# ArnaudPel/CamKifu

Measured on AMD Instinct MI355X. Metric: frames/sec on 1920x1080 video + 19x19 stone-grid match % vs reference SGF, higher is better.
Workload: dtype u8+f16x2(f32 accumulate); 1 GPU; 1920x1080 synthetic game film, 256-frame batches resident in HBM, K1-K12 per ...; cnn=f16x2, frames_per_gpu=256, height=1080, width=1920, parallelism=frames of one video dealt x1, lanes_per_gpu=2, batches_in_flight=2

## Files before the change

camkifu_amd/csrc/k_contours.hip:

```cpp
#include <math.h>

#include <algorithm>

#include "ck_common.h"

#include "ck_uf.h"

#pragma clang fp contract(off)

namespace {

constexpr int MAXC_LIMIT = 1 << 17;
constexpr int PEAK_CAP = 1 << 14;
constexpr int NUMANGLE = 180;

struct FrameTab {
    int n_edges;
    int n_border;
    int n_roots;
    int n_hough_pts;
    int n_peaks;
    int overflow;
    int runs_overflow;
    int pad1;
// ... 150 lines not shown
    for (int i = bx * 256 + threadIdx.x; i < ne + h; i += LIST_BLOCKS * 256) {
        if (i < ne) {
            const int p = E[i];
            L[p] = uf_find(L, p);
            if (!e[p + 1]) L[p + 1] = uf_find(L, p + 1);
        } else {
            const int q = (i - ne) * w;
            L[q] = uf_find(L, q);
        }
    }
}

__device__ __forceinline__ bool in_s0(const int32_t* L, int q, int root0)
{
    return L[L[q]] == root0;
}

__device__ __forceinline__ void claim_root(int f, size_t off, int p, int32_t* __restrict__ compid, FrameTab* __restrict__ tab, int maxc,
                                           int32_t* __restrict__ roots, int32_t* __restrict__ aabb)
{
    const int slot = atomicAdd(&tab[f].n_roots, 1);
    if (slot >= maxc) { tab[f].overflow = 1; compid[off + p] = -1; return; }
    compid[off + p] = slot;
    int32_t* fr = roots + (size_t)f * maxc;
    fr[slot] = p;
    int32_t* bb = aabb + ((size_t)f * maxc + slot) * 4;
    bb[0] = 0x7fffffff; bb[1] = -1; bb[2] = 0x7fffffff; bb[3] = -1;
}

__global__ __launch_bounds__(256) void roots_list_kernel(int h, int w, const int32_t* __restrict__ labels,
                                                         int32_t* __restrict__ compid, FrameTab* __restrict__ tab, int maxc,
                                                         int32_t* __restrict__ roots, int32_t* __restrict__ aabb,
                                                         const int32_t* __restrict__ elist)
{
    int f, bx;
    list_frame_block(LIST_BLOCKS, f, bx);
    const int ne = tab[f].n_edges;
    const size_t off = (size_t)f * h * w;
    const int32_t* L = labels + off;
    const int32_t* E = elist + off;
    const int root0 = L[0];
    for (int i = bx * 256 + threadIdx.x; i < ne; i += LIST_BLOCKS * 256) {
        const int p = E[i];
        if (L[p] != p) continue;
        if (!in_s0(L, p - 1, root0)) continue;
        claim_root(f, off, p, compid, tab, maxc, roots, aabb);
    }
}

__device__ __forceinline__ void grow_boxes(bool b, int cslot, int p, int w, int f, int maxc, int32_t* __restrict__ aabb)
{
    unsigned long long todo = __builtin_amdgcn_ballot_w64(b);
    const int y = p / w, x = p - y * w;
    const int lane = threadIdx.x & 63;
    while (todo) {
        const int lead = __builtin_ctzll(todo);
        const int s_lead = __builtin_amdgcn_readlane(cslot, lead);
        const bool mine = b && cslot == s_lead;
        todo &= ~__builtin_amdgcn_ballot_w64(mine);
        int mnx = mine ? x : 0x7fffffff, mxx = mine ? x : -1, mny = mine ? y : 0x7fffffff, mxy = mine ? y : -1;
#pragma unroll
        for (int d = 32; d >= 1; d >>= 1) {
            mnx = min(mnx, __shfl_xor(mnx, d)); mxx = max(mxx, __shfl_xor(mxx, d));
            mny = min(mny, __shfl_xor(mny, d)); mxy = max(mxy, __shfl_xor(mxy, d));
        }
        if (lane == lead) {
            int32_t* bb = aabb + ((size_t)f * maxc + s_lead) * 4;
            if (mnx < uf_load(bb, 0)) atomicMin(bb + 0, mnx);
            if (mxx > uf_load(bb, 1)) atomicMax(bb + 1, mxx);
            if (mny < uf_load(bb, 2)) atomicMin(bb + 2, mny);
            if (mxy > uf_load(bb, 3)) atomicMax(bb + 3, mxy);
        }
    }
}

__global__ __launch_bounds__(256) void border_list_kernel(const uint8_t* __restrict__ ez, int h, int w,
                                                          const int32_t* __restrict__ labels, const int32_t* __restrict__ compid,
                                                          int maxc, FrameTab* __restrict__ tab, int32_t* __restrict__ aabb,
                                                          const int32_t* __restrict__ elist, int32_t* __restrict__ blist)
{
    int f, bx;
    list_frame_block(LIST_BLOCKS, f, bx);
    const int ne = tab[f].n_edges;
    const size_t off = (size_t)f * h * w;
    const uint8_t* e = ez + off;
    const int32_t* L = labels + off;
    const int32_t* E = elist + off;
    int32_t* B = blist + off;
    const int root0 = L[0];
    const int trips = (ne + LIST_BLOCKS * 256 - 1) / (LIST_BLOCKS * 256);
    for (int t = 0; t < trips; t++) {
        const int i = t * LIST_BLOCKS * 256 + bx * 256 + threadIdx.x;
        bool b = false;
        int p = 0, cslot = -1;
        if (i < ne) {
            p = E[i];
            const int q[4] = { p - 1, p + 1, p - w, p + w };
            int ev[4], head[4], top[4];
#pragma unroll
            for (int k = 0; k < 4; k++) ev[k] = e[q[k]];
#pragma unroll
            for (int k = 0; k < 4; k++) head[k] = L[ev[k] ? 0 : q[k]];
#pragma unroll
            for (int k = 0; k < 4; k++) top[k] = L[head[k]];
#pragma unroll
            for (int k = 0; k < 4; k++) b |= !ev[k] && top[k] == root0;
            if (b) {
                cslot = compid[off + L[p]];
                if ((unsigned)cslot >= (unsigned)maxc) b = false;
            }
        }
        grow_boxes(b, cslot, p, w, f, maxc, aabb);
        const int slot = wave_append(&tab[f].n_border, b);
        if (b) B[slot] = p;
    }
}

struct RunTab {
    unsigned long long* bits;
    uint16_t* rank;
    int32_t* rowbase;
    int32_t* rp;
    int w64;
    int cap_e;
    size_t rp_stride;
};

__device__ __forceinline__ bool rt_edge(const unsigned long long* __restrict__ bf, int w64, int y, int x)
{
    return (bf[(size_t)y * w64 + (x >> 6)] >> (x & 63)) & 1ull;
}
__device__ __forceinline__ int rt_run(const unsigned long long* __restrict__ bf, const uint16_t* __restrict__ rk,
                                      const int32_t* __restrict__ rb, int h, int w64, int y, int x)
{
    const size_t wi = (size_t)y * w64 + (x >> 6);
    const int r = (int)rk[wi] + __builtin_popcountll(bf[wi] & ((1ull << (x & 63)) - 1ull));
    return r ? h + rb[y] + r - 1 : y;
}

__device__ __forceinline__ unsigned long long row16_or(unsigned long long v)
{
    uint32_t lo = (uint32_t)v, hi = (uint32_t)(v >> 32);
#define CK_DPP_OR(CTRL)                                                                   \
    lo |= (uint32_t)__builtin_amdgcn_update_dpp(0, (int)lo, CTRL, 0xf, 0xf, true);       \
    hi |= (uint32_t)__builtin_amdgcn_update_dpp(0, (int)hi, CTRL, 0xf, 0xf, true);
    CK_DPP_OR(0xB1)
    CK_DPP_OR(0x4E)
    CK_DPP_OR(0x141)
    CK_DPP_OR(0x140)
#undef CK_DPP_OR
    return ((unsigned long long)hi << 32) | lo;
}

template <int NS>
__global__ __launch_bounds__(256) void prep_runs_kernel(const uint8_t* __restrict__ edges, int h, int w, int32_t* __restrict__ L,
                                                        FrameTab* __restrict__ tab, int32_t* __restrict__ elist, RunTab rt,
                                                        const int* __restrict__ canny_border_flag)
{
    const int lane = threadIdx.x & 63, wv = threadIdx.x >> 6;
    const int y = blockIdx.x * 4 + wv;
    const int f = blockIdx.y;
    const bool row_live = y < h;
    __shared__ int wtotal[4], wbase;
    const bool keep_edge_parents = canny_border_flag != nullptr && canny_border_flag[f] == 0;
    const size_t off = ((size_t)f * h + y) * w;
    const bool row_inner = y > 0 && y < h - 1;
    int32_t* E = elist + (size_t)f * h * w;
    int32_t* rp = rt.rp + (size_t)f * rt.rp_stride;
    const unsigned long long lt = (1ull << lane) - 1ull;
    uint32_t v[NS];
#pragma unroll
    for (int s = 0; s < NS; s++) {
        const int x = 256 * s + 4 * lane;
        v[s] = 0;
        if (x < w && row_inner && row_live) v[s] = *reinterpret_cast<const uint32_t*>(edges + off + x);
    }
    int nib[NS], before[NS];
    int total = 0;
#pragma unroll
    for (int s = 0; s < NS; s++) {
        const int x = 256 * s + 4 * lane;
        int nb = ((v[s] & 0xFFu) ? 1 : 0) | ((v[s] & 0xFF00u) ? 2 : 0) | ((v[s] & 0xFF0000u) ? 4 : 0) | ((v[s] & 0xFF000000u) ? 8 : 0);
        if (x == 0) nb &= ~1;
        if (x + 3 == w - 1) nb &= ~8;
        nib[s] = nb;
        before[s] = total;
        if (__builtin_amdgcn_ballot_w64(nb != 0)) {
            const unsigned long long b0 = __builtin_amdgcn_ballot_w64(nb & 1), b1 = __builtin_amdgcn_ballot_w64(nb & 2);
            const unsigned long long b2 = __builtin_amdgcn_ballot_w64(nb & 4), b3 = __builtin_amdgcn_ballot_w64(nb & 8);
            before[s] += __builtin_popcountll(b0 & lt) + __builtin_popcountll(b1 & lt) +
                         __builtin_popcountll(b2 & lt) + __builtin_popcountll(b3 & lt);
            total += __builtin_popcountll(b0) + __builtin_popcountll(b1) + __builtin_popcountll(b2) + __builtin_popcountll(b3);
        }
    }
    if (lane == 0) wtotal[wv] = total;
    __syncthreads();
    if (threadIdx.x == 0) {
        const int all = wtotal[0] + wtotal[1] + wtotal[2] + wtotal[3];
        wbase = all ? atomicAdd(&tab[f].n_edges, all) : 0;
    }
    __syncthreads();
    if (!row_live) return;
    int base = wbase;
    for (int kk = 0; kk < wv; kk++) base += wtotal[kk];
    base = __builtin_amdgcn_readfirstlane(base);
    const bool nodes_fit = base + total <= rt.cap_e;
    if (!nodes_fit && lane == 0) tab[f].runs_overflow = 1;
    if (lane == 0) {
        rt.rowbase[(size_t)f * h + y] = base;
        rp[y] = 0;
    }
    unsigned long long* bw = rt.bits + ((size_t)f * h + y) * rt.w64;
    uint16_t* rw = rt.rank + ((size_t)f * h + y) * rt.w64;
#pragma unroll
    for (int s = 0; s < NS; s++) {
        const int x = 256 * s + 4 * lane;
        const int nb = nib[s];
        const unsigned long long word = row16_or((unsigned long long)nb << (4 * (lane & 15)));
        if (x < w) {
            if ((lane & 15) == 0) {
                bw[4 * s + (lane >> 4)] = word;
                rw[4 * s + (lane >> 4)] = (uint16_t)before[s];
            }
            if (nb) {
                int slot = base + before[s];
#pragma unroll
                for (int k = 0; k < 4; k++)
                    if (nb & (1 << k)) {
                        const int p = y * w + x + k;
                        E[slot] = p;
                        if (nodes_fit) rp[h + slot] = slot == base + total - 1 ? 0 : h + slot;
                        if (!keep_edge_parents) L[(size_t)f * h * w + p] = p;
                        slot++;
                    }
            }
        }
    }
}

__global__ __launch_bounds__(256) void link_runs_kernel(int h, int w, int32_t* __restrict__ labels, const FrameTab* __restrict__ tab,
                                                        const int32_t* __restrict__ elist, RunTab rt,
                                                        const int* __restrict__ canny_border_flag)
{
    int f, bx;
    list_frame_block(LIST_BLOCKS, f, bx);
    if (tab[f].runs_overflow) return;
    const bool edges_linked = canny_border_flag != nullptr && canny_border_flag[f] == 0;
    const int ne = tab[f].n_edges, w64 = rt.w64;
    int32_t* L = labels + (size_t)f * h * w;
    const int32_t* E = elist + (size_t)f * h * w;
    const unsigned long long* bf = rt.bits + (size_t)f * h * w64;
    const uint16_t* rk = rt.rank + (size_t)f * h * w64;
    const int32_t* rb = rt.rowbase + (size_t)f * h;
    int32_t* rp = rt.rp + (size_t)f * rt.rp_stride;
    for (int i = bx * 256 + threadIdx.x; i < ne; i += LIST_BLOCKS * 256) {
        const int p = E[i];
        const int y = p / w, x = p - y * w;
        const bool e_n = rt_edge(bf, w64, y - 1, x), e_ne = rt_edge(bf, w64, y - 1, x + 1);
        const bool e_e = rt_edge(bf, w64, y, x + 1), e_s = rt_edge(bf, w64, y + 1, x), e_se = rt_edge(bf, w64, y + 1, x + 1);
        if (!edges_linked) {
            if (rt_edge(bf, w64, y, x - 1)) uf_union(L, p, p - 1);
            if (e_n) uf_union(L, p, p - w);
            else {
                if (rt_edge(bf, w64, y - 1, x - 1)) uf_union(L, p, p - w - 1);
                if (e_ne) uf_union(L, p, p - w + 1);
            }
        }
        if (!e_e && !e_ne) uf_union(rp, h + i, rt_run(bf, rk, rb, h, w64, y - 1, x + 1));
        if (!e_se && !e_e && !e_s) uf_union(rp, rt_run(bf, rk, rb, h, w64, y + 1, x + 1), h + i);
    }
}

__global__ __launch_bounds__(256) void flatten_runs_kernel(int h, int w, int32_t* __restrict__ labels, const FrameTab* __restrict__ tab,
                                                           const int32_t* __restrict__ elist, RunTab rt,
                                                           const int* __restrict__ canny_border_flag)
{
    int f, bx;
    list_frame_block(LIST_BLOCKS, f, bx);
    if (tab[f].runs_overflow) return;
    const bool edges_flat = canny_border_flag != nullptr && canny_border_flag[f] == 0;
    const int ne = tab[f].n_edges;
    int32_t* L = labels + (size_t)f * h * w;
    const int32_t* E = elist + (size_t)f * h * w;
    int32_t* rp = rt.rp + (size_t)f * rt.rp_stride;
    for (int i = bx * 256 + threadIdx.x; i < ne + h; i += LIST_BLOCKS * 256) {
        rp[i] = uf_find(rp, i);
        if (!edges_flat && i < ne) { const int p = E[i]; L[p] = uf_find(L, p); }
    }
}

__global__ __launch_bounds__(256) void roots_runs_kernel(int h, int w, const int32_t* __restrict__ labels,
                                                         int32_t* __restrict__ compid, FrameTab* __restrict__ tab, int maxc,
                                                         int32_t* __restrict__ roots, int32_t* __restrict__ aabb,
                                                         const int32_t* __restrict__ elist, RunTab rt)
{
    int f, bx;
    list_frame_block(LIST_BLOCKS, f, bx);
    if (tab[f].runs_overflow) return;
    const int ne = tab[f].n_edges;
    const size_t off = (size_t)f * h * w;
    const int32_t* L = labels + off;
    const int32_t* E = elist + off;
    const int32_t* rb = rt.rowbase + (size_t)f * h;
    const int32_t* rp = rt.rp + (size_t)f * rt.rp_stride;
    const int root0 = rp[0];
    for (int i = bx * 256 + threadIdx.x; i < ne; i += LIST_BLOCKS * 256) {
        const int p = E[i];
        if (L[p] != p) continue;
        const int y = p / w;
        const int west = (i == rb[y]) ? y : h + i - 1;
        if (rp[west] != root0) continue;
        claim_root(f, off, p, compid, tab, maxc, roots, aabb);
    }
}

__global__ __launch_bounds__(256) void border_runs_kernel(int h, int w, const int32_t* __restrict__ labels,
                                                          const int32_t* __restrict__ compid, int maxc, FrameTab* __restrict__ tab,
                                                          int32_t* __restrict__ aabb, const int32_t* __restrict__ elist,
                                                          int32_t* __restrict__ blist, RunTab rt)
{
    int f, bx;
    list_frame_block(LIST_BLOCKS, f, bx);
    if (tab[f].runs_overflow) return;
    const int ne = tab[f].n_edges, w64 = rt.w64;
    const size_t off = (size_t)f * h * w;
    const int32_t* L = labels + off;
    const int32_t* E = elist + off;
    int32_t* B = blist + off;
    const unsigned long long* bf = rt.bits + (size_t)f * h * w64;
    const uint16_t* rk = rt.rank + (size_t)f * h * w64;
    const int32_t* rb = rt.rowbase + (size_t)f * h;
    const int32_t* rp = rt.rp + (size_t)f * rt.rp_stride;
    const int root0 = rp[0];
    const int trips = (ne + LIST_BLOCKS * 256 - 1) / (LIST_BLOCKS * 256);
    for (int t = 0; t < trips; t++) {
        const int i = t * LIST_BLOCKS * 256 + bx * 256 + threadIdx.x;
        bool b = false;
        int p = 0, cslot = -1;
        if (i < ne) {
            p = E[i];
            const int y = p / w, x = p - y * w;
            const size_t wi = (size_t)y * w64 + (x >> 6);
            const unsigned long long here = bf[wi];
            const bool e_w = (x & 63) ? (here >> ((x & 63) - 1)) & 1ull : rt_edge(bf, w64, y, x - 1);
            const bool e_e = ((x & 63) != 63) ? (here >> ((x & 63) + 1)) & 1ull : rt_edge(bf, w64, y, x + 1);
            const bool e_n = rt_edge(bf, w64, y - 1, x), e_s = rt_edge(bf, w64, y + 1, x);
            const int n_w = (i == rb[y]) ? y : h + i - 1;
            const int n_e = h + i;
            const int n_n = e_n ? 0 : rt_run(bf, rk, rb, h, w64, y - 1, x);
            const int n_s = e_s ? 0 : rt_run(bf, rk, rb, h, w64, y + 1, x);
            const int t_w = rp[e_w ? 0 : n_w], t_e = rp[e_e ? 0 : n_e], t_n = rp[n_n], t_s = rp[n_s];
            b = (!e_w && t_w == root0) || (!e_e && t_e == root0) || (!e_n && t_n == root0) || (!e_s && t_s == root0);
            if (b) {
                cslot = compid[off + L[p]];
                if ((unsigned)cslot >= (unsigned)maxc) b = false;
            }
        }
        grow_boxes(b, cslot, p, w, f, maxc, aabb);
        const int slot = wave_append(&tab[f].n_border, b);
        if (b) B[slot] = p;
    }
}

__global__ void pack_tables_kernel(const int32_t* __restrict__ roots, const int32_t* __restrict__ aabb, int maxc, int k, int n,
                                   int32_t* __restrict__ out )
{
    const int i = blockIdx.x * blockDim.x + threadIdx.x;
    if (i >= n * k) return;
    const int f = i / k, s = i % k;
    out[i] = roots[(size_t)f * maxc + s];
    const int32_t* bb = aabb + ((size_t)f * maxc + s) * 4;
    int32_t* ob = out + (size_t)n * k + (size_t)i * 4;
    ob[0] = bb[0]; ob[1] = bb[1]; ob[2] = bb[2]; ob[3] = bb[3];
}

__global__ void pack_peaks_kernel(const int32_t* __restrict__ peaks, int k, int n, int32_t* __restrict__ out)
{
    const int i = blockIdx.x * blockDim.x + threadIdx.x;
    if (i >= n * k) return;
    const int f = i / k, s = i % k;
    out[2 * (size_t)i] = peaks[((size_t)f * PEAK_CAP + s) * 2];
    out[2 * (size_t)i + 1] = peaks[((size_t)f * PEAK_CAP + s) * 2 + 1];
}

__device__ __forceinline__ bool mid_of_run(const uint8_t* e, int p, int w)
{
    return (e[p - 1] && e[p + 1]) || (e[p - w] && e[p + w]) ||
           (e[p - w - 1] && e[p + w + 1]) || (e[p - w + 1] && e[p + w - 1]);
}

__device__ __forceinline__ bool mid_of_run_raw(const uint8_t* e, int p, int w, int h)
{
    const int y = p / w, x = p - y * w;
    auto at = [&](int dy, int dx) {
        const int yy = y + dy, xx = x + dx;
        return xx > 0 && xx < w - 1 && yy > 0 && yy < h - 1 && e[yy * w + xx] != 0;
    };
    return (at(0, -1) && at(0, 1)) || (at(-1, 0) && at(1, 0)) || (at(-1, -1) && at(1, 1)) || (at(-1, 1) && at(1, -1));
}

__device__ __forceinline__ bool hull_candidate(const uint8_t* __restrict__ ez, size_t off, int p, int w, int h, int raw)
{
    return !(raw ? mid_of_run_raw(ez + off, p, w, h) : mid_of_run(ez + off, p, w));
}

__global__ __launch_bounds__(256) void gather_points_kernel(const uint8_t* __restrict__ ez, int h, int w,
                                                            const int32_t* __restrict__ labels, const int32_t* __restrict__ compid,
                                                            int maxc, const uint8_t* __restrict__ want, int wpitch, const FrameTab* __restrict__ tab,
                                                            const int32_t* __restrict__ blist, int32_t* __restrict__ counter, int cap,
                                                            int32_t* __restrict__ pts ,
                                                            int raw )
{
    int f, bx;
    list_frame_block(LIST_BLOCKS, f, bx);
    const int nb = tab[f].n_border;
    const size_t off = (size_t)f * h * w;
    const int32_t* B = blist + off;
    const int trips = (nb + LIST_BLOCKS * 256 - 1) / (LIST_BLOCKS * 256);
    for (int t = 0; t < trips; t++) {
        const int i = t * LIST_BLOCKS * 256 + bx * 256 + threadIdx.x;
        bool take = false;
        int p = 0, slot = 0;
// ... 195 lines not shown
    list_frame_block(LIST_BLOCKS, f, bx);
    if (!sel[f * 4 + 3]) return;
    const int nb = tab[f].n_border;
    const size_t off = (size_t)f * h * w;
    const int32_t* B = blist + off;
    const int s0 = sel[f * 4], s1 = sel[f * 4 + 1], s2 = sel[f * 4 + 2];
    for (int i = bx * 256 + threadIdx.x; i < nb; i += LIST_BLOCKS * 256) {
        const int p = B[i];
        const int slot = compid[off + labels[off + p]];
        if (slot != s0 && slot != s1 && slot != s2) continue;
        if (ghost) ghost[off + p] = 255;
        const int k = atomicAdd(&tab[f].n_hough_pts, 1);
        const int y = p / w, x = p - y * w;
        if (k < pcap) hpts[(size_t)f * pcap + k] = (uint32_t)x | ((uint32_t)y << 16);
        else tab[f].overflow = 1;
    }
}

__global__ __launch_bounds__(HOUGH_THREADS) void hough_vote_peaks_kernel(const uint32_t* __restrict__ hpts, FrameTab* __restrict__ tab,
                                                               int pcap, const float* __restrict__ trig ,
                                                               int numrho, int rb, int threshold,
                                                               int32_t* __restrict__ peaks )
{
#pragma clang fp contract(off)
    extern __shared__ __attribute__((aligned(16))) uint32_t slab16[];
    const int f = blockIdx.y;
    const int nthreads = blockDim.x;
    const int n0 = blockIdx.x * rb;
    const int stride = numrho + 2;
    const int rowdw = (stride + 1) >> 1;
    const int nrows = rb + 2;
    for (int i = threadIdx.x; i < nrows * rowdw; i += nthreads) slab16[i] = 0u;
    __syncthreads();
    int npts = tab[f].n_hough_pts;
    if (npts > pcap) npts = pcap;
    const uint32_t* P = hpts + (size_t)f * pcap;
    const int half = (numrho - 1) / 2;
    const int j_lo = n0 == 0 ? 1 : 0;
    int j_hi = NUMANGLE - (n0 - 1);
    if (j_hi > nrows) j_hi = nrows;
    for (int i = threadIdx.x; i < npts; i += nthreads) {
        const uint32_t pk = P[i];
        const float xf = (float)(pk & 0xFFFF), yf = (float)(pk >> 16);
        for (int j = j_lo; j < j_hi; j++) {
            const int n = n0 - 1 + j;
            const float a = xf * trig[n];
            const float b = yf * trig[NUMANGLE + n];
            const float s = a + b;
            const int c = (int)rintf(s) + half + 1;
            atomicAdd(&slab16[j * rowdw + (c >> 1)], 1u << (16 * (c & 1)));
        }
    }
    __syncthreads();
    const uint16_t* cnt = reinterpret_cast<const uint16_t*>(slab16);
    const int rowhw = 2 * rowdw;
    for (int k = 0; k < rb; k++) {
        const int n = n0 + k;
        if (n >= NUMANGLE) break;
        const uint16_t* row = cnt + (k + 1) * rowhw;
        const uint32_t* roww = slab16 + (k + 1) * rowdw;
        for (int d = threadIdx.x; d < rowdw; d += nthreads) {
            const uint32_t two = roww[d];
            if ((int)(two & 0xFFFFu) <= threshold && (int)(two >> 16) <= threshold) continue;
#pragma unroll
            for (int hlf = 0; hlf < 2; hlf++) {
                const int c = 2 * d + hlf, r = c - 1;
                if (r < 0 || r >= numrho) continue;
                const int v = hlf ? (int)(two >> 16) : (int)(two & 0xFFFFu);
                if (v <= threshold) continue;
                if (v > row[r] && v >= row[r + 2] && v > row[r + 1 - rowhw] && v >= row[r + 1 + rowhw]) {
                    const int i = atomicAdd(&tab[f].n_peaks, 1);
                    if (i < PEAK_CAP) {
                        peaks[((size_t)f * PEAK_CAP + i) * 2] = (n + 1) * stride + r + 1;
                        peaks[((size_t)f * PEAK_CAP + i) * 2 + 1] = v;
                    } else tab[f].overflow = 1;
                }
            }
        }
    }
}

struct LabelScratch {
    uint8_t* ez;
    int32_t *L, *compid, *elist, *blist;
    FrameTab* d_tab;
    int32_t *d_roots, *d_aabb;
    int maxc;
    size_t fpx, npx, tab_bytes;
    dim3 lgrid;
};

int label_scratch(ck_ctx* ctx, int n, int h, int w, size_t misc_extra, size_t comp_extra, LabelScratch& s)
{
    s.fpx = (size_t)h * w, s.npx = s.fpx * n;
    s.maxc = (int)(s.fpx / 4 + 1);
    if (s.maxc > MAXC_LIMIT) s.maxc = MAXC_LIMIT;
    s.tab_bytes = sizeof(FrameTab) * (size_t)n;
    CK_TRY(ck_ensure(ctx, ctx->ghost, s.npx));
    CK_TRY(ck_ensure(ctx, ctx->labels, s.npx * 4));
    CK_TRY(ck_ensure(ctx, ctx->labels2, s.npx * 4));
    CK_TRY(ck_ensure(ctx, ctx->lists, s.npx * 8));
    CK_TRY(ck_ensure(ctx, ctx->misc, s.tab_bytes + misc_extra + 64));
    CK_TRY(ck_ensure(ctx, ctx->comp, (size_t)n * s.maxc * (4 + 16 + comp_extra)));
    s.ez = (uint8_t*)ctx->ghost.p;
    s.L = (int32_t*)ctx->labels.p;
    s.compid = (int32_t*)ctx->labels2.p;
    s.elist = (int32_t*)ctx->lists.p;
    s.blist = s.elist + s.npx;
    s.d_tab = (FrameTab*)ctx->misc.p;
    s.d_roots = (int32_t*)ctx->comp.p;
    s.d_aabb = s.d_roots + (size_t)n * s.maxc;
    s.lgrid = list_grid(LIST_BLOCKS, n);
    return CK_OK;
}

bool dword_rows(const uint8_t* d_edges, int w) { return (w & 3) == 0 && ((uintptr_t)d_edges & 3) == 0; }

int label_dense(ck_ctx* ctx, const uint8_t* d_edges, int n, int h, int w, const LabelScratch& s)
{
    const dim3 lblock(256);
    CK_HIP(ctx, hipMemsetAsync(s.d_tab, 0, s.tab_bytes, ctx->stream));
    if (dword_rows(d_edges, w))
        hipLaunchKernelGGL(prep_rows4_kernel, dim3((h + 3) / 4, n), dim3(256), 0, ctx->stream, d_edges, h, w, s.ez, s.L, s.d_tab, s.elist);
    else
        hipLaunchKernelGGL(prep_rows_kernel, dim3((h + 3) / 4, n), dim3(256), 0, ctx->stream, d_edges, h, w, s.ez, s.L, s.d_tab, s.elist);
    hipLaunchKernelGGL(link_list_kernel, s.lgrid, lblock, 0, ctx->stream, (const uint8_t*)s.ez, h, w, s.L,
                       (const FrameTab*)s.d_tab, (const int32_t*)s.elist);
    hipLaunchKernelGGL(flatten_list_kernel, s.lgrid, lblock, 0, ctx->stream, (const uint8_t*)s.ez, h, w, s.L,
                       (const FrameTab*)s.d_tab, (const int32_t*)s.elist);
    hipLaunchKernelGGL(roots_list_kernel, s.lgrid, lblock, 0, ctx->stream, h, w, (const int32_t*)s.L, s.compid, s.d_tab, s.maxc,
                       s.d_roots, s.d_aabb, (const int32_t*)s.elist);
    hipLaunchKernelGGL(border_list_kernel, s.lgrid, lblock, 0, ctx->stream, (const uint8_t*)s.ez, h, w, (const int32_t*)s.L,
                       (const int32_t*)s.compid, s.maxc, s.d_tab, s.d_aabb, (const int32_t*)s.elist, s.blist);
    CK_HIP(ctx, hipGetLastError());
    return CK_OK;
}

int label_runs(ck_ctx* ctx, const uint8_t* d_edges, int n, int h, int w, const LabelScratch& s, const int* kflag)
{
    const dim3 lblock(256);
    CK_HIP(ctx, hipMemsetAsync(s.d_tab, 0, s.tab_bytes, ctx->stream));
    RunTab rt;
    rt.w64 = (w + 63) / 64;
    const size_t cap_e = std::min(s.fpx, std::max(s.fpx / 4, (size_t)1 << 16));
    rt.cap_e = (int)cap_e;
    rt.rp_stride = cap_e + (size_t)h;
    const size_t bits_b = (size_t)n * h * rt.w64 * 8, rank_b = (size_t)n * h * rt.w64 * 2, rb_b = (size_t)n * h * 4;
    const size_t rank_o = bits_b, rb_o = (rank_o + rank_b + 15) & ~(size_t)15, rp_o = (rb_o + rb_b + 15) & ~(size_t)15;
    CK_TRY(ck_ensure(ctx, ctx->runs, rp_o + (size_t)n * rt.rp_stride * 4));
    rt.bits = (unsigned long long*)ctx->runs.p;
    rt.rank = (uint16_t*)((char*)ctx->runs.p + rank_o);
    rt.rowbase = (int32_t*)((char*)ctx->runs.p + rb_o);
    rt.rp = (int32_t*)((char*)ctx->runs.p + rp_o);
    if (w <= 1024)
        hipLaunchKernelGGL(prep_runs_kernel<4>, dim3((h + 3) / 4, n), dim3(256), 0, ctx->stream, d_edges, h, w, s.L, s.d_tab, s.elist, rt, kflag);
    else if (w <= 2048)
        hipLaunchKernelGGL(prep_runs_kernel<8>, dim3((h + 3) / 4, n), dim3(256), 0, ctx->stream, d_edges, h, w, s.L, s.d_tab, s.elist, rt, kflag);
    else
        hipLaunchKernelGGL(prep_runs_kernel<16>, dim3((h + 3) / 4, n), dim3(256), 0, ctx->stream, d_edges, h, w, s.L, s.d_tab, s.elist, rt, kflag);
    hipLaunchKernelGGL(link_runs_kernel, s.lgrid, lblock, 0, ctx->stream, h, w, s.L, (const FrameTab*)s.d_tab, (const int32_t*)s.elist, rt, kflag);
    hipLaunchKernelGGL(flatten_runs_kernel, s.lgrid, lblock, 0, ctx->stream, h, w, s.L, (const FrameTab*)s.d_tab, (const int32_t*)s.elist, rt, kflag);
    hipLaunchKernelGGL(roots_runs_kernel, s.lgrid, lblock, 0, ctx->stream, h, w, (const int32_t*)s.L, s.compid, s.d_tab, s.maxc,
                       s.d_roots, s.d_aabb, (const int32_t*)s.elist, rt);
    hipLaunchKernelGGL(border_runs_kernel, s.lgrid, lblock, 0, ctx->stream, h, w, (const int32_t*)s.L, (const int32_t*)s.compid, s.maxc,
                       s.d_tab, s.d_aabb, (const int32_t*)s.elist, s.blist, rt);
    CK_HIP(ctx, hipGetLastError());
    return CK_OK;
}

struct Board {
    ck_ctx* ctx;
    const uint8_t* d_edges;
    int n, h, w;
    HostLap lap;
    LabelScratch s;
    int32_t* d_sel;
    float* d_trig;
    uint8_t* d_want;
    bool run_table;
    std::vector<FrameTab> tab;
    int nc_max;
    std::vector<size_t> first;
    std::vector<int32_t> root;
    std::vector<double> ub, area;
    std::vector<uint8_t> known;

    int fetch_tab()
    {
        CK_HIP(ctx, hipMemcpyAsync(tab.data(), s.d_tab, s.tab_bytes, hipMemcpyDeviceToHost, ctx->stream));
        CK_HIP(ctx, hipStreamSynchronize(ctx->stream));
        return CK_OK;
    }

    int label(const int* d_canny_border_flag)
    {
        run_table = dword_rows(d_edges, w) && w <= 4096;
        auto launch_ccl = [&](bool runs) -> int {
            TimeScope ts(ctx, "ccl");
            return runs ? label_runs(ctx, d_edges, n, h, w, s, d_canny_border_flag) : label_dense(ctx, d_edges, n, h, w, s);
        };
        CK_TRY(launch_ccl(run_table));
        lap("ccl kernels");
        tab.resize((size_t)n);
        CK_TRY(fetch_tab());
        if (run_table) {
            bool redo = false;
            for (int f = 0; f < n; f++) redo = redo || tab[f].runs_overflow;
            if (redo) {
                run_table = false;
                CK_TRY(launch_ccl(false));
                CK_TRY(fetch_tab());
            }
        }
        return CK_OK;
    }

    int tables(ck_board_result* res)
    {
        nc_max = 0;
        first.assign((size_t)n + 1, 0);
        for (int f = 0; f < n; f++) {
            if (tab[f].overflow) return ck_fail(ctx, CK_ERR_CAPACITY, "frame %d: more than %d external contours", f, s.maxc);
            nc_max = std::max(nc_max, tab[f].n_roots);
            first[f + 1] = first[f] + (size_t)tab[f].n_roots;
        }
        std::vector<int32_t> hroots((size_t)n * nc_max), haabb((size_t)n * nc_max * 4);
        if (nc_max) {
            const size_t cnt = (size_t)n * nc_max;
            CK_TRY(ck_ensure(ctx, ctx->pts, cnt * 20 + 64));
            int32_t* d_pack = (int32_t*)ctx->pts.p;
            hipLaunchKernelGGL(pack_tables_kernel, dim3((unsigned)((cnt + 255) / 256)), dim3(256), 0, ctx->stream,
                               (const int32_t*)s.d_roots, (const int32_t*)s.d_aabb, s.maxc, nc_max, n, d_pack);
            CK_HIP(ctx, hipMemcpyAsync(hroots.data(), d_pack, cnt * 4, hipMemcpyDeviceToHost, ctx->stream));
            CK_HIP(ctx, hipMemcpyAsync(haabb.data(), d_pack + cnt, cnt * 16, hipMemcpyDeviceToHost, ctx->stream));
            CK_HIP(ctx, hipStreamSynchronize(ctx->stream));
        }
        const size_t total = first[(size_t)n];
        root.resize(total); ub.resize(total); area.assign(total, 0.0); known.resize(total);
        for (int f = 0; f < n; f++) {
            const int nc = tab[f].n_roots;
            res[f].status = nc == 0 ? CK_BOARD_NO_CONTOUR : CK_BOARD_LINES;
            res[f].n_contours = nc; res[f].n_lines = 0; res[f].reserved = 0; res[f].biggest_area = 0;
            const int32_t* hr = hroots.data() + (size_t)f * nc_max;
            const int32_t* hb = haabb.data() + (size_t)f * nc_max * 4;
            for (int k = 0; k < nc; k++) {
                const double dx = (double)hb[4 * k + 1] - hb[4 * k], dy = (double)hb[4 * k + 3] - hb[4 * k + 2];
                const size_t c = first[f] + k;
                root[c] = hr[k]; ub[c] = dx * dy; known[c] = dx * dy == 0.0;
            }
        }
        lap("tables d2h");
        return CK_OK;
    }

    int gather(const std::vector<uint8_t>& want, int gcap, int32_t* d_pts, int32_t* d_counter, int& npts)
    {
        const dim3 lblock(256);
        const bool raw_edges = run_table;
        const uint8_t* e_img = raw_edges ? d_edges : (const uint8_t*)s.ez;
        {
            TimeScope ts(ctx, "contour_gather");
            CK_HIP(ctx, hipMemcpyAsync(d_want, want.data(), (size_t)n * nc_max, hipMemcpyHostToDevice, ctx->stream));
            const int segcap = gcap / n;
            CK_TRY(ck_ensure(ctx, ctx->accum, (size_t)n * segcap * 8 + (size_t)n * 4 + 64));
            int32_t* d_seg = (int32_t*)ctx->accum.p;
            int32_t* d_fcnt = d_seg + (size_t)n * segcap * 2;
            CK_HIP(ctx, hipMemsetAsync(d_fcnt, 0, (size_t)n * 4, ctx->stream));
            CK_HIP(ctx, hipMemsetAsync(d_counter, 0, 8, ctx->stream));
            hipLaunchKernelGGL(gather_segments_kernel, s.lgrid, lblock, 0, ctx->stream, e_img, h, w,
                               (const int32_t*)s.L, (const int32_t*)s.compid, s.maxc, (const uint8_t*)d_want, nc_max,
                               (const FrameTab*)s.d_tab, (const int32_t*)s.blist, d_fcnt, segcap, d_seg, (int)raw_edges);
            hipLaunchKernelGGL(compact_points_kernel, dim3(n), dim3(256), 0, ctx->stream, (const int32_t*)d_fcnt, n, segcap,
                               (const int32_t*)d_seg, gcap, d_pts, d_counter);
            CK_HIP(ctx, hipGetLastError());
        }
        int two[2] = {0, 0};
        CK_HIP(ctx, hipMemcpyAsync(two, d_counter, 8, hipMemcpyDeviceToHost, ctx->stream));
        CK_HIP(ctx, hipStreamSynchronize(ctx->stream));
        npts = two[0];
        if (two[1]) {
            TimeScope ts(ctx, "contour_gather");
            CK_HIP(ctx, hipMemsetAsync(d_counter, 0, 4, ctx->stream));
            hipLaunchKernelGGL(gather_points_kernel, s.lgrid, lblock, 0, ctx->stream, e_img, h, w,
                               (const int32_t*)s.L, (const int32_t*)s.compid, s.maxc, (const uint8_t*)d_want, nc_max,
                               (const FrameTab*)s.d_tab, (const int32_t*)s.blist, d_counter, gcap, d_pts, (int)raw_edges);
            CK_HIP(ctx, hipGetLastError());
            CK_HIP(ctx, hipMemcpyAsync(&npts, d_counter, 4, hipMemcpyDeviceToHost, ctx->stream));
            CK_HIP(ctx, hipStreamSynchronize(ctx->stream));
        }
        if (npts > gcap) return ck_fail(ctx, CK_ERR_CAPACITY, "too many contour points (%d > %d)", npts, gcap);
        return CK_OK;
    }

    int areas()
    {
        const int gcap = (int)(s.npx < (1u << 22) ? s.npx : (1u << 22));
        CK_TRY(ck_ensure(ctx, ctx->pts, (size_t)gcap * 12 + 64));
        int32_t* d_pts = (int32_t*)ctx->pts.p;
        int32_t* d_counter = d_pts + (size_t)gcap * 3;
        std::vector<uint8_t> want((size_t)n * std::max(nc_max, 1));
        for (int round = 0; round < 3 && nc_max > 0; round++) {
            bool any = false;
            std::fill(want.begin(), want.end(), 0);
            for (int f = 0; f < n; f++) {
                const size_t c = first[f];
                const int nc = (int)(first[f + 1] - c);
                if (ck_board_round_want(round, nc, ub.data() + c, area.data() + c, known.data() + c, want.data() + (size_t)f * nc_max)) any = true;
            }
            if (!any) break;
            if (round == 2) return ck_fail(ctx, CK_ERR_STATE, "contour selection did not converge");
            int npts = 0;
            CK_TRY(gather(want, gcap, d_pts, d_counter, npts));
            std::vector<int32_t> hp((size_t)npts * 2), hf((size_t)npts);
// ... 234 lines not shown
```

Baseline: 23480 frames/s.

## Label edge runs in 32-row LDS bands with local union-find plus seam pass

Replaces the per-row prep kernel and global link kernel with a band kernel that processes 32 rows per 512-thread block. It keeps edge bitmaps, ranks and parent arrays in LDS and does union-find locally with workgroup-scoped atomics. A separate seam kernel then joins components across band boundaries through global union-find. The aim is to cut global atomic traffic and scattered global reads in linking. The cost is heavy LDS use, which limits occupancy, plus a global fallback path when a band has more nodes than fit in LDS.

```diff
diff --git a/camkifu_amd/csrc/k_contours.hip b/camkifu_amd/csrc/k_contours.hip
--- a/camkifu_amd/csrc/k_contours.hip
+++ b/camkifu_amd/csrc/k_contours.hip
@@ -326,122 +326,251 @@
     return ((unsigned long long)hi << 32) | lo;
 }
 
+constexpr int BAND_ROWS = 32, BAND_THREADS = 512, BAND_WAVES = BAND_THREADS / 64, BAND_RPW = BAND_ROWS / BAND_WAVES;
+constexpr int BAND_NODES = 4096;
+
 template <int NS>
-__global__ __launch_bounds__(256) void prep_runs_kernel(const uint8_t* __restrict__ edges, int h, int w, int32_t* __restrict__ L,
+__global__ __launch_bounds__(BAND_THREADS, NS == 16 ? 6 : 8) void band_runs_kernel(const uint8_t* __restrict__ edges, int h, int w, int32_t* __restrict__ L,
                                                         FrameTab* __restrict__ tab, int32_t* __restrict__ elist, RunTab rt,
                                                         const int* __restrict__ canny_border_flag)
 {
+    constexpr int W64 = 4 * NS, CAP = BAND_NODES;
+    constexpr int RC = NS == 16 ? 1 : 2;
+    __shared__ unsigned long long sbits[BAND_ROWS][W64];
+    __shared__ uint16_t srank[BAND_ROWS][W64];
+    __shared__ int par[CAP];
+    __shared__ uint16_t spos[CAP];
+    __shared__ int rowtot[BAND_ROWS], rowoff[BAND_ROWS + 1], sbase;
     const int lane = threadIdx.x & 63, wv = threadIdx.x >> 6;
-    const int y = blockIdx.x * 4 + wv;
-    const int f = blockIdx.y;
-    const bool row_live = y < h;
-    __shared__ int wtotal[4], wbase;
+    const int y0 = blockIdx.x * BAND_ROWS, f = blockIdx.y;
+    const int nrows = min(BAND_ROWS, h - y0);
     const bool keep_edge_parents = canny_border_flag != nullptr && canny_border_flag[f] == 0;
-    const size_t off = ((size_t)f * h + y) * w;
-    const bool row_inner = y > 0 && y < h - 1;
-    int32_t* E = elist + (size_t)f * h * w;
+    const size_t foff = (size_t)f * h * w;
+    int32_t* E = elist + foff;
     int32_t* rp = rt.rp + (size_t)f * rt.rp_stride;
     const unsigned long long lt = (1ull << lane) - 1ull;
-    uint32_t v[NS];
-#pragma unroll
-    for (int s = 0; s < NS; s++) {
-        const int x = 256 * s + 4 * lane;
-        v[s] = 0;
-        if (x < w && row_inner && row_live) v[s] = *reinterpret_cast<const uint32_t*>(edges + off + x);
-    }
-    int nib[NS], before[NS];
-    int total = 0;
-#pragma unroll
-    for (int s = 0; s < NS; s++) {
-        const int x = 256 * s + 4 * lane;
-        int nb = ((v[s] & 0xFFu) ? 1 : 0) | ((v[s] & 0xFF00u) ? 2 : 0) | ((v[s] & 0xFF0000u) ? 4 : 0) | ((v[s] & 0xFF000000u) ? 8 : 0);
-        if (x == 0) nb &= ~1;
-        if (x + 3 == w - 1) nb &= ~8;
-        nib[s] = nb;
-        before[s] = total;
-        if (__builtin_amdgcn_ballot_w64(nb != 0)) {
-            const unsigned long long b0 = __builtin_amdgcn_ballot_w64(nb & 1), b1 = __builtin_amdgcn_ballot_w64(nb & 2);
-            const unsigned long long b2 = __builtin_amdgcn_ballot_w64(nb & 4), b3 = __builtin_amdgcn_ballot_w64(nb & 8);
-            before[s] += __builtin_popcountll(b0 & lt) + __builtin_popcountll(b1 & lt) +
-                         __builtin_popcountll(b2 & lt) + __builtin_popcountll(b3 & lt);
-            total += __builtin_popcountll(b0) + __builtin_popcountll(b1) + __builtin_popcountll(b2) + __builtin_popcountll(b3);
-        }
-    }
-    if (lane == 0) wtotal[wv] = total;
+    const int sh = 4 * (lane & 15), wq = lane >> 4;
+
+#pragma unroll
+    for (int k0 = 0; k0 < BAND_RPW; k0 += RC) {
+        uint32_t v[RC][NS];
+#pragma unroll
+        for (int c = 0; c < RC; c++) {
+            const int r = wv * BAND_RPW + k0 + c, y = y0 + r;
+            const bool live = r < nrows && y > 0 && y < h - 1;
+#pragma unroll
+            for (int s = 0; s < NS; s++) {
+                const int x = 256 * s + 4 * lane;
+                v[c][s] = 0;
+                if (x < w && live) v[c][s] = *reinterpret_cast<const uint32_t*>(edges + foff + (size_t)y * w + x);
+            }
+        }
+#pragma unroll
+        for (int c = 0; c < RC; c++) {
+            const int r = wv * BAND_RPW + k0 + c, y = y0 + r;
+            unsigned long long* bw = rt.bits + ((size_t)f * h + y) * rt.w64;
+            uint16_t* rw = rt.rank + ((size_t)f * h + y) * rt.w64;
+            int total = 0;
+#pragma unroll
+            for (int s = 0; s < NS; s++) {
+                const int x = 256 * s + 4 * lane;
+                const uint32_t vv = v[c][s];
+                int nb = ((vv & 0xFFu) ? 1 : 0) | ((vv & 0xFF00u) ? 2 : 0) | ((vv & 0xFF0000u) ? 4 : 0) | ((vv & 0xFF000000u) ? 8 : 0);
+                if (x == 0) nb &= ~1;
+                if (x + 3 == w - 1) nb &= ~8;
+                int before = total;
+                if (__builtin_amdgcn_ballot_w64(nb != 0)) {
+                    const unsigned long long b0 = __builtin_amdgcn_ballot_w64(nb & 1), b1 = __builtin_amdgcn_ballot_w64(nb & 2);
+                    const unsigned long long b2 = __builtin_amdgcn_ballot_w64(nb & 4), b3 = __builtin_amdgcn_ballot_w64(nb & 8);
+                    before += __builtin_popcountll(b0 & lt) + __builtin_popcountll(b1 & lt) +
+                              __builtin_popcountll(b2 & lt) + __builtin_popcountll(b3 & lt);
+                    total += __builtin_popcountll(b0) + __builtin_popcountll(b1) + __builtin_popcountll(b2) + __builtin_popcountll(b3);
+                }
+                const unsigned long long word = row16_or((unsigned long long)nb << sh);
+                if (x < w && r < nrows && (lane & 15) == 0) {
+                    bw[4 * s + wq] = word;
+                    rw[4 * s + wq] = (uint16_t)before;
+                    sbits[r][4 * s + wq] = word;
+                    srank[r][4 * s + wq] = (uint16_t)before;
+                }
+            }
+            if (lane == 0) rowtot[r] = total;
+        }
+    }
     __syncthreads();
-    if (threadIdx.x == 0) {
-        const int all = wtotal[0] + wtotal[1] + wtotal[2] + wtotal[3];
-        wbase = all ? atomicAdd(&tab[f].n_edges, all) : 0;
+
+    if (wv == 0) {
+        const int t = lane < BAND_ROWS ? rowtot[lane] : 0;
+        int inc = t;
+#pragma unroll
+        for (int d = 1; d < BAND_ROWS; d <<= 1) {
+            const int o = __shfl_up(inc, d);
+            if (lane >= d) inc += o;
+        }
+        if (lane < BAND_ROWS) rowoff[lane] = inc - t;
+        if (lane == BAND_ROWS - 1) {
+            rowoff[BAND_ROWS] = inc;
+            sbase = inc ? atomicAdd(&tab[f].n_edges, inc) : 0;
+        }
     }
     __syncthreads();
-    if (!row_live) return;
-    int base = wbase;
-    for (int kk = 0; kk < wv; kk++) base += wtotal[kk];
-    base = __builtin_amdgcn_readfirstlane(base);
-    const bool nodes_fit = base + total <= rt.cap_e;
-    if (!nodes_fit && lane == 0) tab[f].runs_overflow = 1;
-    if (lane == 0) {
-        rt.rowbase[(size_t)f * h + y] = base;
-        rp[y] = 0;
-    }
-    unsigned long long* bw = rt.bits + ((size_t)f * h + y) * rt.w64;
-    uint16_t* rw = rt.rank + ((size_t)f * h + y) * rt.w64;
-#pragma unroll
-    for (int s = 0; s < NS; s++) {
-        const int x = 256 * s + 4 * lane;
-        const int nb = nib[s];
-        const unsigned long long word = row16_or((unsigned long long)nb << (4 * (lane & 15)));
-        if (x < w) {
-            if ((lane & 15) == 0) {
-                bw[4 * s + (lane >> 4)] = word;
-                rw[4 * s + (lane >> 4)] = (uint16_t)before[s];
-            }
-            if (nb) {
-                int slot = base + before[s];
-#pragma unroll
-                for (int k = 0; k < 4; k++)
-                    if (nb & (1 << k)) {
-                        const int p = y * w + x + k;
-                        E[slot] = p;
-                        if (nodes_fit) rp[h + slot] = slot == base + total - 1 ? 0 : h + slot;
-                        if (!keep_edge_parents) L[(size_t)f * h * w + p] = p;
-                        slot++;
+    const int ne_b = rowoff[BAND_ROWS], base = sbase;
+    const bool nodes_fit = base + ne_b <= rt.cap_e;
+    const bool lds_fit = ne_b < CAP;
+    if (!nodes_fit && threadIdx.x == 0) tab[f].runs_overflow = 1;
+    if (threadIdx.x == 0) { par[0] = 0; if (nodes_fit && !lds_fit) rp[0] = 0; }
+    for (int k = 0; k < BAND_RPW; k++) {
+        const int r = wv * BAND_RPW + k, y = y0 + r;
+        if (r >= nrows) break;
+        const int ro = rowoff[r], rend = rowoff[r + 1];
+        if (lane == 0) {
+            rt.rowbase[(size_t)f * h + y] = base + ro;
+            if (nodes_fit) rp[y] = 0;
+        }
+        if (rend == ro) continue;
+#pragma unroll
+        for (int s = 0; s < NS; s++) {
+            const int x = 256 * s + 4 * lane;
+            if (x >= w) continue;
+            const unsigned long long word = sbits[r][4 * s + wq];
+            const int nb = (int)(word >> sh) & 15;
+            if (!nb) continue;
+            int j = ro + (int)srank[r][4 * s + wq] + __builtin_popcountll(word & ((1ull << sh) - 1ull));
+#pragma unroll
+            for (int kk = 0; kk < 4; kk++)
+                if (nb & (1 << kk)) {
+                    const int p = y * w + x + kk;
+                    E[base + j] = p;
+                    const bool last = j == rend - 1;
+                    if (nodes_fit) {
+                        if (lds_fit) {
+                            par[1 + j] = last ? 0 : 1 + j;
+                            spos[j] = (uint16_t)((x + kk) | ((r & 15) << 12));
+                        } else rp[h + base + j] = last ? 0 : h + base + j;
                     }
-            }
-        }
-    }
-}
-
-__global__ __launch_bounds__(256) void link_runs_kernel(int h, int w, int32_t* __restrict__ labels, const FrameTab* __restrict__ tab,
+                    if (!keep_edge_parents && nodes_fit && !lds_fit) L[foff + p] = p;
+                    j++;
+                }
+        }
+    }
+    if (!nodes_fit) return;
+    if (!lds_fit) __threadfence();
+    __syncthreads();
+
+    auto lbit = [&](int r, int x) { return (sbits[r][x >> 6] >> (x & 63)) & 1ull; };
+    auto lidx = [&](int r, int x) {
+        return (int)srank[r][x >> 6] + __builtin_popcountll(sbits[r][x >> 6] & ((1ull << (x & 63)) - 1ull));
+    };
+    if (lds_fit) {
+        auto lfind = [&](int a) {
+            int p = __hip_atomic_load(par + a, __ATOMIC_RELAXED, __HIP_MEMORY_SCOPE_WORKGROUP);
+            while (p != a) { a = p; p = __hip_atomic_load(par + a, __ATOMIC_RELAXED, __HIP_MEMORY_SCOPE_WORKGROUP); }
+            return a;
+        };
+        auto lunion = [&](int a, int b) {
+            for (;;) {
+                a = lfind(a); b = lfind(b);
+                if (a == b) return;
+                if (a < b) { const int t = a; a = b; b = t; }
+                const int old = atomicMin(par + a, b);
+                if (old == a) return;
+                a = old;
+            }
+        };
+        auto lrun = [&](int r, int x) { const int k = lidx(r, x); return k ? rowoff[r] + k : 0; };
+        const int half = rowoff[16];
+        auto lrow = [&](int j) { return (spos[j] >> 12) | (j >= half ? 16 : 0); };
+        for (int j = threadIdx.x; j < ne_b; j += BAND_THREADS) {
+            const int x = spos[j] & 4095, r = lrow(j);
+            if (lbit(r, x + 1)) continue;
+            if (r > 0 && !lbit(r - 1, x + 1)) lunion(1 + j, lrun(r - 1, x + 1));
+            if (r < nrows - 1 && !lbit(r + 1, x + 1) && !lbit(r + 1, x)) lunion(lrun(r + 1, x + 1), 1 + j);
+        }
+        __syncthreads();
+        for (int j = threadIdx.x; j < ne_b; j += BAND_THREADS) {
+            const int root = lfind(1 + j);
+            rp[h + base + j] = root ? h + base + root - 1 : 0;
+        }
+        if (keep_edge_parents) return;
+        __syncthreads();
+        for (int j = threadIdx.x; j < ne_b; j += BAND_THREADS) par[1 + j] = 1 + j;
+        __syncthreads();
+        auto lnode = [&](int r, int x) { return 1 + rowoff[r] + lidx(r, x); };
+        for (int j = threadIdx.x; j < ne_b; j += BAND_THREADS) {
+            const int x = spos[j] & 4095, r = lrow(j);
+            if (lbit(r, x - 1)) lunion(1 + j, j);
+            if (r > 0) {
+                if (lbit(r - 1, x)) lunion(1 + j, lnode(r - 1, x));
+                else {
+                    if (lbit(r - 1, x - 1)) lunion(1 + j, lnode(r - 1, x - 1));
+                    if (lbit(r - 1, x + 1)) lunion(1 + j, lnode(r - 1, x + 1));
+                }
+            }
+        }
+        __syncthreads();
+        for (int j = threadIdx.x; j < ne_b; j += BAND_THREADS) {
+            const int t = lfind(1 + j) - 1;
+            L[foff + (size_t)(y0 + lrow(j)) * w + (spos[j] & 4095)] = (y0 + lrow(t)) * w + (spos[t] & 4095);
+        }
+    } else {
+        auto grun = [&](int r, int x) { const int k = lidx(r, x); return k ? h + base + rowoff[r] + k - 1 : y0 + r; };
+        for (int j = threadIdx.x; j < ne_b; j += BAND_THREADS) {
+            const int p = uf_load(E, base + j);
+            const int y = p / w, x = p - y * w, r = y - y0;
+            if (!keep_edge_parents) {
+                int32_t* Lf = L + foff;
+                if (lbit(r, x - 1)) uf_union(Lf, p, p - 1);
+                if (r > 0) {
+                    if (lbit(r - 1, x)) uf_union(Lf, p, p - w);
+                    else {
+                        if (lbit(r - 1, x - 1)) uf_union(Lf, p, p - w - 1);
+                        if (lbit(r - 1, x + 1)) uf_union(Lf, p, p - w + 1);
+                    }
+                }
+            }
+            if (lbit(r, x + 1)) continue;
+            if (r > 0 && !lbit(r - 1, x + 1)) uf_union(rp, h + base + j, grun(r - 1, x + 1));
+            if (r < nrows - 1 && !lbit(r + 1, x + 1) && !lbit(r + 1, x)) uf_union(rp, grun(r + 1, x + 1), h + base + j);
+        }
+    }
+}
+
+__global__ __launch_bounds__(256) void seam_runs_kernel(int h, int w, int32_t* __restrict__ labels, const FrameTab* __restrict__ tab,
                                                         const int32_t* __restrict__ elist, RunTab rt,
                                                         const int* __restrict__ canny_border_flag)
 {
-    int f, bx;
-    list_frame_block(LIST_BLOCKS, f, bx);
+    const int f = blockIdx.y, yb = (blockIdx.x + 1) * BAND_ROWS;
     if (tab[f].runs_overflow) return;
     const bool edges_linked = canny_border_flag != nullptr && canny_border_flag[f] == 0;
-    const int ne = tab[f].n_edges, w64 = rt.w64;
+    const int w64 = rt.w64;
     int32_t* L = labels + (size_t)f * h * w;
     const int32_t* E = elist + (size_t)f * h * w;
     const unsigned long long* bf = rt.bits + (size_t)f * h * w64;
     const uint16_t* rk = rt.rank + (size_t)f * h * w64;
     const int32_t* rb = rt.rowbase + (size_t)f * h;
     int32_t* rp = rt.rp + (size_t)f * rt.rp_stride;
-    for (int i = bx * 256 + threadIdx.x; i < ne; i += LIST_BLOCKS * 256) {
-        const int p = E[i];
-        const int y = p / w, x = p - y * w;
-        const bool e_n = rt_edge(bf, w64, y - 1, x), e_ne = rt_edge(bf, w64, y - 1, x + 1);
-        const bool e_e = rt_edge(bf, w64, y, x + 1), e_s = rt_edge(bf, w64, y + 1, x), e_se = rt_edge(bf, w64, y + 1, x + 1);
-        if (!edges_linked) {
-            if (rt_edge(bf, w64, y, x - 1)) uf_union(L, p, p - 1);
-            if (e_n) uf_union(L, p, p - w);
+    auto row_count = [&](int y) {
+        const size_t wi = (size_t)y * w64 + w64 - 1;
+        return (int)rk[wi] + __builtin_popcountll(bf[wi]);
+    };
+    const int nu = row_count(yb - 1), nl = row_count(yb);
+    for (int i = threadIdx.x; i < nu + nl; i += 256) {
+        const bool lower = i >= nu;
+        const int y = lower ? yb : yb - 1;
+        const int slot = rb[y] + (lower ? i - nu : i);
+        const int p = E[slot], x = p - y * w;
+        if (lower && !edges_linked) {
+            if (rt_edge(bf, w64, y - 1, x)) uf_union(L, p, p - w);
             else {
                 if (rt_edge(bf, w64, y - 1, x - 1)) uf_union(L, p, p - w - 1);
-                if (e_ne) uf_union(L, p, p - w + 1);
-            }
-        }
-        if (!e_e && !e_ne) uf_union(rp, h + i, rt_run(bf, rk, rb, h, w64, y - 1, x + 1));
-        if (!e_se && !e_e && !e_s) uf_union(rp, rt_run(bf, rk, rb, h, w64, y + 1, x + 1), h + i);
+                if (rt_edge(bf, w64, y - 1, x + 1)) uf_union(L, p, p - w + 1);
+            }
+        }
+        if (rt_edge(bf, w64, y, x + 1)) continue;
+        if (lower) {
+            if (!rt_edge(bf, w64, y - 1, x + 1)) uf_union(rp, h + slot, rt_run(bf, rk, rb, h, w64, y - 1, x + 1));
+        } else if (!rt_edge(bf, w64, y + 1, x + 1) && !rt_edge(bf, w64, y + 1, x))
+            uf_union(rp, rt_run(bf, rk, rb, h, w64, y + 1, x + 1), h + slot);
     }
 }
 
@@ -943,13 +1072,16 @@
     rt.rank = (uint16_t*)((char*)ctx->runs.p + rank_o);
     rt.rowbase = (int32_t*)((char*)ctx->runs.p + rb_o);
     rt.rp = (int32_t*)((char*)ctx->runs.p + rp_o);
+    const int nbands = (h + BAND_ROWS - 1) / BAND_ROWS;
     if (w <= 1024)
-        hipLaunchKernelGGL(prep_runs_kernel<4>, dim3((h + 3) / 4, n), dim3(256), 0, ctx->stream, d_edges, h, w, s.L, s.d_tab, s.elist, rt, kflag);
+        hipLaunchKernelGGL(band_runs_kernel<4>, dim3(nbands, n), dim3(BAND_THREADS), 0, ctx->stream, d_edges, h, w, s.L, s.d_tab, s.elist, rt, kflag);
     else if (w <= 2048)
-        hipLaunchKernelGGL(prep_runs_kernel<8>, dim3((h + 3) / 4, n), dim3(256), 0, ctx->stream, d_edges, h, w, s.L, s.d_tab, s.elist, rt, kflag);
+        hipLaunchKernelGGL(band_runs_kernel<8>, dim3(nbands, n), dim3(BAND_THREADS), 0, ctx->stream, d_edges, h, w, s.L, s.d_tab, s.elist, rt, kflag);
     else
-        hipLaunchKernelGGL(prep_runs_kernel<16>, dim3((h + 3) / 4, n), dim3(256), 0, ctx->stream, d_edges, h, w, s.L, s.d_tab, s.elist, rt, kflag);
-    hipLaunchKernelGGL(link_runs_kernel, s.lgrid, lblock, 0, ctx->stream, h, w, s.L, (const FrameTab*)s.d_tab, (const int32_t*)s.elist, rt, kflag);
+        hipLaunchKernelGGL(band_runs_kernel<16>, dim3(nbands, n), dim3(BAND_THREADS), 0, ctx->stream, d_edges, h, w, s.L, s.d_tab, s.elist, rt, kflag);
+    if (nbands > 1)
+        hipLaunchKernelGGL(seam_runs_kernel, dim3(nbands - 1, n), dim3(256), 0, ctx->stream, h, w, s.L, (const FrameTab*)s.d_tab,
+                           (const int32_t*)s.elist, rt, kflag);
     hipLaunchKernelGGL(flatten_runs_kernel, s.lgrid, lblock, 0, ctx->stream, h, w, s.L, (const FrameTab*)s.d_tab, (const int32_t*)s.elist, rt, kflag);
     hipLaunchKernelGGL(roots_runs_kernel, s.lgrid, lblock, 0, ctx->stream, h, w, (const int32_t*)s.L, s.compid, s.d_tab, s.maxc,
                        s.d_roots, s.d_aabb, (const int32_t*)s.elist, rt);
```

Result: slower. 22810 frames/s (-2.8%).
